# hellobertrand/zxc

Measured on NVIDIA H100. Metric: decompress GB/s (uncompressed), higher is better.
Workload: dtype u8

## Files before the change

profiles/occupancy_probe.py:

```python
import argparse
import ctypes as C
import os
import re
import shutil
import subprocess
import sys
import tempfile
import time

ROOT = os.path.dirname(os.path.dirname(os.path.abspath(__file__)))
sys.path.insert(0, os.path.join(ROOT, "tests"))
sys.path.insert(0, ROOT)

VARIANTS = [
    ("parent", "parent", "", {}, "shipped: lean at 8 CTAs, 64 registers without spills"),
    ("cta7", "cta7", "-DLEAN_CTAS_PER_SM=7u", {}, "the same source built for 7 CTAs (72 registers)"),
    ("grid7", "parent", "", {"ZXC_B200_DECODE_CTAS": "7"},
     "the shipped build with a 7-CTA grid: the eighth CTA alone, at the 164 KB carve-out"),
    ("pad7", "pad7", "-DLEAN_CTAS_PER_SM=7u -DLEAN_SMEM_PAD=2048u", {},
     "7 CTAs, 164 KB carve-out: the L1 shrink alone"),
    ("ring2k_7", "ring2k_7", "-DRING_BYTES=2048u -DLEAN_CTAS_PER_SM=7u", {}, "7 CTAs, 2 KiB rings"),
    ("ring2k_8", "ring2k_8", "-DRING_BYTES=2048u", {}, "8 CTAs, 2 KiB rings: more warps at a 100 KB carve-out"),
]
LEAN = "_Z17zxc_decode_kernelILb0ELb0ELb0ELb1EEv12DecodeParams"


def build(out_dir, nvextra):
    lib = os.path.join(out_dir, "libzxc.so.4")
    if not os.path.exists(lib):
        subprocess.run(["make", "-j", str(os.cpu_count() or 4), f"NVEXTRA={nvextra}", f"OUT={out_dir}"],
                       cwd=os.path.join(ROOT, "zxc_b200", "csrc"), check=True, stdout=subprocess.DEVNULL)
    return lib


def lean_resources(out_dir):
    log = open(os.path.join(out_dir, "obj", "ptxas.log")).read()
    blk = log.split(f"Compiling entry function '{LEAN}'")[1].split("Compiling entry function")[0]
    sp = re.search(r"(\d+) bytes spill stores, (\d+) bytes spill loads", blk)
    return int(re.search(r"Used (\d+) registers", blk).group(1)), int(sp.group(1)), int(sp.group(2))


def card():
    q = "name,power.limit,clocks.max.sm,clocks.sm"
    r = subprocess.run(["nvidia-smi", f"--query-gpu={q}", "--format=csv,noheader"], stdout=subprocess.PIPE, text=True)
    return r.stdout.strip().splitlines()[0] if r.returncode == 0 and r.stdout.strip() else "nvidia-smi unavailable"


class Runner:
    def __init__(self, path, dev, d_src, d_dst, d_jobs, d_status, nb):
        import bench
        import torch

        lib = C.CDLL(path)
        lib.zxc_b200_decode_scratch_size.restype = C.c_size_t
        lib.zxc_b200_decode_scratch_size.argtypes = [C.c_uint32]
        lib.zxc_b200_decode_blocks.restype = C.c_int
        lib.zxc_b200_decode_blocks.argtypes = [C.c_void_p, C.c_void_p, C.c_void_p, C.c_uint32, C.c_void_p,
                                               C.c_void_p, C.c_uint32, C.c_void_p, C.c_void_p, C.c_size_t,
                                               C.c_uint32, C.c_int, C.c_void_p]
        self.lib, self.nb, self.block = lib, nb, bench.BLOCK
        self.bufs = (d_src, d_dst, d_jobs, d_status)
        self.scratch_size = lib.zxc_b200_decode_scratch_size(bench.BLOCK)
        self.d_scratch = torch.empty(self.scratch_size, dtype=torch.uint8, device=dev)
        self.stream = torch.cuda.current_stream(dev)
        lean, general = C.c_int(0), C.c_int(0)
        assert lib.zxc_b200_decode_occupancy(C.byref(lean), C.byref(general)) == 0
        self.occupancy = (lean.value, general.value)

# ... 103 lines not shown
```

zxc_b200/csrc/zxc_decode.cuh:

```cuda
#pragma once
#include <cuda_runtime.h>
#include <stdint.h>

#include <type_traits>

#include "zxc_b200.h"
#include "zxc_error.h"

typedef uint8_t u8;
typedef uint32_t u32;
typedef uint64_t u64;
typedef int32_t i32;

#define FULL 0xFFFFFFFFu
#ifndef ZXC_FASTMOD
#define ZXC_FASTMOD 1
#endif
#ifndef ZXC_TAIL_SMEM
#define ZXC_TAIL_SMEM 1
#endif
#ifndef ZXC_ALIGNED_LD
#define ZXC_ALIGNED_LD 1
#endif
#ifndef ZXC_HINTS
// ... 96 lines not shown
__device__ __forceinline__ u8* ring_at(u32 a) { return reinterpret_cast<u8*>(__cvta_shared_to_generic((size_t)opaque(a))); }
__device__ __forceinline__ u32 grid_warp_now() {
    u32 t, c;
    asm volatile("mov.u32 %0, %%tid.x;" : "=r"(t));
    asm volatile("mov.u32 %0, %%ctaid.x;" : "=r"(c));
    return c * WARPS_PER_CTA + (t >> 5);
}
#else
extern u8 smem[];
static inline u32 smem_addr(const void* p) { return (u32)(reinterpret_cast<const u8*>(p) - smem); }
static inline u32 opaque(u32 v) { return v; }
static inline u8* ring_at(u32 a) { return smem + a; }
static inline u32 grid_warp_now() { return blockIdx.x * WARPS_PER_CTA + (threadIdx.x >> 5); }
template <int OFF> static inline void sts32(u32 a, u32 v) { memcpy(smem + a + OFF, &v, 4); }
template <int OFF> static inline void sts16(u32 a, u32 v) { const unsigned short h = (unsigned short)v; memcpy(smem + a + OFF, &h, 2); }
template <int OFF> static inline void sts8(u32 a, u32 v) { smem[a + OFF] = (u8)v; }
#endif

#ifdef __CUDACC__
__device__ __forceinline__ void prefetch_l1(const void* p) { asm volatile("prefetch.global.L1 [%0];" ::"l"(p)); }
#else
static inline void prefetch_l1(const void*) {}
#endif

#if ZXC_TRACE
#define TRACE_SLOTS 16
#define TRACE_ROWS 8192
enum {
    TR_UNPACK, TR_SCAN, TR_LIT, TR_MATCH, TR_TAIL, TR_FLUSH, TR_START, TR_END, TR_GIANT, TR_CLAIM,
    TR_BATCHES, TR_BLOCKS, TR_M_RING, TR_M_GLOBAL, TR_M_DICT, TR_M_SEQ
};
__device__ unsigned long long zxc_trace_acc[TRACE_ROWS * TRACE_SLOTS];
__device__ __forceinline__ void trace_add(u32 slot, unsigned long long v, u32 lane) {
    const u32 row = blockIdx.x * WARPS_PER_CTA + (threadIdx.x >> 5);
    if (lane == 0 && row < TRACE_ROWS) atomicAdd(&zxc_trace_acc[row * TRACE_SLOTS + slot], v);
}
#define ZXC_TRACE_DECL long long tr_t = clock64()
#define ZXC_TRACE_MARK(slot, lane)                               \
    do {                                                         \
        const long long tr_n = clock64();                        \
        trace_add(slot, (unsigned long long)(tr_n - tr_t), lane); \
        tr_t = tr_n;                                             \
    } while (0)
#define ZXC_TRACE_ADD(slot, v, lane) trace_add(slot, (unsigned long long)(v), lane)
#else
#define ZXC_TRACE_DECL
#define ZXC_TRACE_MARK(slot, lane)
#define ZXC_TRACE_ADD(slot, v, lane)
#endif

#include "zxc_decode_stage.cuh"
#define WARP_SMEM_BYTES (RING_BYTES + STAGE_BYTES)
#define DECODE_SMEM_BYTES (WARPS_PER_CTA * WARP_SMEM_BYTES)

#include "zxc_huffman.cuh"

__host__ __device__ __forceinline__ u32 scr_lit_cap(u32 bs) { return (bs + 255u) & ~255u; }
__host__ __device__ __forceinline__ u32 scr_tok_cap(u32 bs) { return (bs / 4u + 64u + 255u) & ~255u; }
__host__ __device__ __forceinline__ u32 scr_cum_cap(u32 bs) {
    return (11u * (scr_lit_cap(bs) / 8u) + 4u * 512u + 255u) & ~255u;
}
__host__ __device__ __forceinline__ u32 scr_stride(u32 bs) {
    return 256u + scr_lit_cap(bs) + scr_tok_cap(bs) + (u32)HUF_WORK_BYTES + scr_cum_cap(bs);
}

__device__ __forceinline__ void warp_copy(u8* d, const u8* s, u32 n, u32 lane) {
    u32 k = lane;
    for (; k + 96 < n; k += 128) {
        const u8 a = s[k], b = s[k + 32], c = s[k + 64], e = s[k + 96];
        d[k] = a;
        d[k + 32] = b;
        d[k + 64] = c;
        d[k + 96] = e;
    }
    for (; k < n; k += 32) d[k] = s[k];
}

__device__ __forceinline__ u32 read_varint(const u8* e, u32& pos, u32 end) {
    if (pos >= end) return 0;
    const u32 b0 = e[pos];
    if (b0 < 0x80) {
        pos += 1;
        return b0;
    }
    if (b0 < 0xC0) {
        if (pos + 1 >= end) {
            pos = end;
            return 0;
        }
        const u32 v = (b0 & 0x3F) | ((u32)e[pos + 1] << 6);
        pos += 2;
        return v;
    }
    if (b0 < 0xE0) {
        if (pos + 2 >= end) {
            pos = end;
            return 0;
        }
        const u32 v = (b0 & 0x1F) | ((u32)e[pos + 1] << 5) | ((u32)e[pos + 2] << 13);
        pos += 3;
        return v;
    }
    pos = end;
    return 0;
}

// ... 383 lines not shown
    const u32 total = __shfl_sync(FULL, incl, 31);
    const u32 excl = incl - c;
    const u32 pk = (my_d & (RING_BYTES - 1)) | (my_n << 16);
    const unsigned long long my_sp64 = reinterpret_cast<unsigned long long>(my_sp);
    for (u32 base = 0; base < total; base += 32) {
        ZXC_STAT(8, 1);
        const u32 q = base + lane;
        const bool act = q < total;
        u32 lo = 0, hi = 31;
#pragma unroll
        for (int it = 0; it < 5; it++) {
            const u32 mid = (lo + hi) >> 1;
            const u32 v = __shfl_sync(FULL, incl, mid);
            if (v > q) hi = mid;
            else lo = mid + 1;
        }
        const u32 j = lo & 31u;
        const u32 k = q - __shfl_sync(FULL, excl, j);
        const u32 pj = __shfl_sync(FULL, pk, j);
        const u8* sp = reinterpret_cast<const u8*>(__shfl_sync(FULL, my_sp64, j));
        if (act) {
            const u32 da = pj & 3u;
            const u32 n = pj >> 16;
            const u32 lfe = (da + n) >> 2;
            const u32 w0 = (da ? 1u : 0u) + 4u * k;
            const u8* bp = sp - da;
            const u32 m = (u32)(reinterpret_cast<uintptr_t>(bp)) & 3u;
            const u32* wp = reinterpret_cast<const u32*>(bp - m) + w0;
            const u32 dw = ring_s + (pj & 0xFFFFu) - da + 4u * w0;
            const u32 sh = m * 8u;
            const u32 left = lfe - w0;
            const u32 nsrc = left + (m ? 1u : 0u);
            u32 W[5];
#pragma unroll
            for (int i = 0; i < 5; i++) W[i] = (u32)i < nsrc ? wp[i] : 0u;
            sts32<0>(dw, __funnelshift_r(W[0], W[1], sh));
            if (1 < left) sts32<4>(dw, __funnelshift_r(W[1], W[2], sh));
            if (2 < left) sts32<8>(dw, __funnelshift_r(W[2], W[3], sh));
            if (3 < left) sts32<12>(dw, __funnelshift_r(W[3], W[4], sh));
        }
    }
}

#ifndef ZXC_NW
#define ZXC_NW 8
#endif
#define LIT_SHORT (4u * ZXC_NW - 4u)
#define MATCH_SHORT (4u * ZXC_NW - 4u)

__device__ __forceinline__ u32* esc_table(u8* scratch, u32 block_cap) {
    return reinterpret_cast<u32*>(scratch + scr_lit_cap(block_cap) + scr_tok_cap(block_cap) + (u32)HUF_WORK_BYTES);
}

template <bool UNITS, bool GHI, bool HAS_DICT, bool LEAN>
__device__ int decode_lz_block(const u8* pay, u32 comp, u8* out, u32 cap, const u8* dict_in,
                               u32 dict_size_in, const u8* dict_huf, u8* scratch, u32 scratch_cap, u8* ring,
                               u32 lane, const DecodeParams& P) {
    constexpr bool ghi = GHI;
    const u8* dict = HAS_DICT ? dict_in : (const u8*)0;
    const u32 dict_size = HAS_DICT ? dict_size_in : 0u;
    ZXC_TRACE_DECL;
    ZXC_TRACE_ADD(TR_BLOCKS, 1, lane);
    Sections S;
    const int prc = parse_sections<LEAN>(pay, comp, ghi, cap, dict_huf, scratch, scratch_cap, lane, S);
    if (prc != ZXC_OK) return prc;
    const u8* lit = S.lit;
    const u8* tok = S.tok;
    const u8* offs = S.offs;
    const u8* ext = S.ext;
    const u32 ext_end = S.ext_end, n_lit_avail = S.n_lit_avail, n_seq = S.n_seq, enc_off = S.enc_off;

    if (UNITS && cap <= 65536u) {
        u8* tok_buf = scratch + scr_lit_cap(scratch_cap);
        u8* hw_area = tok_buf + scr_tok_cap(scratch_cap);
        const bool scratch_busy = (lit == scratch) || (tok == tok_buf);
        u8* tab = scratch_busy ? hw_area : scratch;
        const u32 tab_bytes = scratch_busy ? (u32)HUF_WORK_BYTES + scr_cum_cap(scratch_cap)
                                           : scr_stride(scratch_cap) - 256u;
        const int r = decode_lz_units(lit, n_lit_avail, tok, offs, ext, ext_end, n_seq, enc_off, ghi, out, cap, dict,
                                      dict_size, tab, tab_bytes, lane);
        if (r != UW_NOT_TAKEN) return r;
    }

    const u32 mask = RING_BYTES - 1;
    const u32 esc = ghi ? 255u : 15u;
    const u32 lt_mask = (1u << lane) - 1u;
    const bool al16 = (reinterpret_cast<uintptr_t>(out) & 15u) == 0;
    Window w;
    w.ring = ring;
    w.out = out;
    w.dict = dict;
    w.dict_size = dict_size;
    w.near_lo = 0;
    const u32 ring_s = smem_addr(ring);
    (void)ring_s;
#define W_RING()                                     \
    do {                                             \
        if constexpr (LEAN) w.ring = ring_at(ring_s); \
    } while (0)
    u32 O = 0, L = 0, F = 0, epos = 0, ring_lo = 0;

    u32* vals = esc_table(scratch, scratch_cap);
    if constexpr (LEAN) {
        if (4ull * ext_end > scr_cum_cap(scratch_cap)) return D2_DEFER_STATUS;
    }
    const bool use_vals = LEAN || (ext_end != 0u && 4ull * ext_end <= scr_cum_cap(scratch_cap));
    u32 n_val = 0, ord_base = 0;
    if (use_vals && (!LEAN || ext_end != 0u)) {
        const u32 seg = max(4u, (ext_end + 31u) / 32u);
        const u32 nseg = (ext_end + seg - 1u) / seg;
        const u32 lo = lane * seg, hi = min(ext_end, lo + seg);
        u64 inc = lane < nseg ? z2_seg_map(ext, lo, hi, ext_end) : Z2_MAP_ID;
#pragma unroll
        for (int dd = 1; dd < 32; dd <<= 1) {
            const u64 o = __shfl_up_sync(FULL, inc, dd);
            if (lane >= (u32)dd) inc = z2_map_compose(o, inc);
        }
        u64 excl = __shfl_up_sync(FULL, inc, 1);
        if (lane == 0) excl = Z2_MAP_ID;
        n_val = z2_map_cnt(__shfl_sync(FULL, inc, 31), 0);
        if (lane < nseg) {
            const u32 ent = z2_map_exit(excl, 0);
            if (ent != 3u) z2_seg_values(ext, lo, hi, ext_end, ent, z2_map_cnt(excl, 0), vals);
        }
        __syncwarp();
    }

#if ZXC_STAGE
    const u32 stage_s = smem_addr(ring) + RING_BYTES;
    TokStream::open(stage_s, tok, (ghi ? 4u : 1u) * n_seq, pay + comp, tok >= pay && tok < pay + comp);
    OffStream::open(stage_s, ghi ? tok : offs, ghi ? 0u : (enc_off ? 1u : 2u) * n_seq, pay + comp, !ghi);
#if ZXC_STAGE_LIT
    LitStream::open(stage_s, lit, n_lit_avail, pay + comp, lit >= pay && lit < pay + comp);
#define ST_LIT_CLOSE() LitStream::close(stage_s)
#else
#define ST_LIT_CLOSE() do { } while (0)
#endif
#define ST_CLOSE()                   \
    do {                             \
        TokStream::close(stage_s);   \
        OffStream::close(stage_s);   \
        ST_LIT_CLOSE();              \
    } while (0)
#else
#define ST_CLOSE() do { } while (0)
#define ST_LIT_CLOSE() do { } while (0)
#endif

    ZXC_TRACE_MARK(TR_START, lane);

    u32 base = 0;
    while (base < n_seq) {
        const u32 i = base + lane;
        const bool valid = i < n_seq;
        u32 ll = 0, ml = 0, off = 1;
        if (LEAN && !HAS_DICT && lane < 4u && L + 128u * lane < n_lit_avail) prefetch_l1(lit + L + 128u * lane);
#if ZXC_STAGE
        const u32 tok_w = ghi ? 4u : 1u, off_w = enc_off ? 1u : 2u;
        const u32 tx0 = (u32)(reinterpret_cast<uintptr_t>(tok) & 15u), ox0 = (u32)(reinterpret_cast<uintptr_t>(offs) & 15u);
        const u32 i_end = min(base + 32u, n_seq);
        const StWindow st_t = TokStream::need(stage_s, tok, tx0 + tok_w * base, tx0 + tok_w * i_end, 0u, lane);
        const StWindow st_o = OffStream::need(stage_s, offs, ox0 + off_w * base, ox0 + off_w * i_end, 0u, lane);
        const bool t_st = tx0 + tok_w * i_end <= st_t.hi, o_st = !ghi && ox0 + off_w * i_end <= st_o.hi;
#endif
        if (valid) {
            u32 a, b = 0;
#if ZXC_STAGE
            if (!ghi) {
                a = t_st ? lds8(st_t.ring_s + ((tx0 + i) & (ST_RING - 1u))) : (u32)tok[i];
                if (!o_st) {
                    b = enc_off ? (u32)offs[i] : ld16(offs + 2 * (size_t)i);
                } else if (enc_off) {
                    b = lds8(st_o.ring_s + ((ox0 + i) & (ST_RING - 1u)));
                } else {
                    const u32 x = ox0 + 2u * i;
                    b = (ox0 & 1u) ? (lds8(st_o.ring_s + (x & (ST_RING - 1u))) |
                                      (lds8(st_o.ring_s + ((x + 1u) & (ST_RING - 1u))) << 8))
                                   : lds16(st_o.ring_s + (x & (ST_RING - 1u)));
                }
            } else if (t_st) {
                const u32 x = tx0 + 4u * i;
                if (tx0 & 3u) {
                    a = lds8(st_t.ring_s + (x & (ST_RING - 1u))) | (lds8(st_t.ring_s + ((x + 1u) & (ST_RING - 1u))) << 8) |
                        (lds8(st_t.ring_s + ((x + 2u) & (ST_RING - 1u))) << 16) |
                        (lds8(st_t.ring_s + ((x + 3u) & (ST_RING - 1u))) << 24);
                } else {
                    a = lds32(st_t.ring_s + (x & (ST_RING - 1u)));
                }
            } else {
                a = ld32(tok + 4 * (size_t)i);
            }
#else
            if (!ghi) {
                const u8* tk = tok;
                if constexpr (LEAN) tk = lit + opaque(n_lit_avail);
                a = tk[i];
#if ZXC_ALIGNED_LD
                if (LEAN) {
                    const u32 oi = n_seq + (enc_off ? i : 2u * i);
                    if (enc_off) b = (u32)tk[oi];
                    else if ((reinterpret_cast<uintptr_t>(tk) + n_seq) & 1u) b = ld16(tk + oi);
                    else b = (u32)*reinterpret_cast<const unsigned short*>(tk + oi);
                } else if (enc_off) b = (u32)offs[i];
                else if (reinterpret_cast<uintptr_t>(offs) & 1u) b = ld16(offs + 2 * (size_t)i);
                else b = (u32)reinterpret_cast<const unsigned short*>(offs)[i];
#else
                b = enc_off ? (u32)offs[i] : ld16(offs + 2 * (size_t)i);
#endif
            } else {
#if ZXC_ALIGNED_LD
                a = (reinterpret_cast<uintptr_t>(tok) & 3u) ? ld32(tok + 4 * (size_t)i) : reinterpret_cast<const u32*>(tok)[i];
#else
                a = ld32(tok + 4 * (size_t)i);
#endif
            }
#endif
            if (!ghi) {
                ll = a >> 4;
                ml = a & 15;
                off = b + 1;
            } else {
                ll = a >> 24;
                ml = (a >> 16) & 0xFF;
                off = (a & 0xFFFF) + 1;
            }
        }
        const bool e_ll = valid && ll == esc, e_ml = valid && ml == esc;
        const u32 m_ll = __ballot_sync(FULL, e_ll), m_ml = __ballot_sync(FULL, e_ml);
        ZXC_TRACE_MARK(TR_UNPACK, lane);
        u32 k_esc = 0, epos_end = epos;
        if ((m_ll | m_ml) && use_vals) {
            const u32* vt = vals;
            if constexpr (LEAN) vt = esc_table(warp_scratch(P, grid_warp_now()), P.block_cap);
            u32 k = ord_base + __popc(m_ll & lt_mask) + __popc(m_ml & lt_mask);
            if (e_ll) {
                ll += k < n_val ? vt[k] : 0u;
                k++;
            }
            if (e_ml) ml += k < n_val ? vt[k] : 0u;
        } else if (ZXC_RARE((m_ll | m_ml) != 0)) {
            const u32 ord_ll = __popc(m_ll & lt_mask) + __popc(m_ml & lt_mask);
            k_esc = __popc(m_ll) + __popc(m_ml);
            u32 my_pos = ext_end;
            for (u32 s = 0; s < k_esc; s++) {
                if (s == ord_ll) my_pos = epos_end;
                epos_end = varint_advance(ext, epos_end, ext_end);
            }
            if (e_ll) ll += read_varint(ext, my_pos, ext_end);
            if (e_ml) ml += read_varint(ext, my_pos, ext_end);
        }
        if (valid) ml += 5;
        const u32 tot = ll + ml;
        const u32 s_ll = warp_incl_scan(ll, lane);
        const u32 s_tot = warp_incl_scan(tot, lane);

        const u32 nvalid = min(32u, n_seq - base);
        const u32 m = __popc(__ballot_sync(FULL, valid && s_tot <= RING_LIMIT));
        const u32 lit_start = L + s_ll - ll;
        const u32 out_start = O + s_tot - tot;
        const u32 mdst = out_start + ll;

        if (ZXC_RARE(m == 0)) {
            const u32 g_ll = __shfl_sync(FULL, ll, 0), g_ml = __shfl_sync(FULL, ml, 0),
                      g_off = __shfl_sync(FULL, off, 0);
            ZXC_STAT(9, 1);
            if (L + g_ll > n_lit_avail || (u64)O + g_ll + g_ml > cap) {
                ST_CLOSE();
                return ZXC_ERROR_OVERFLOW;
            }
            if (O + g_ll + dict_size < g_off) {
                ST_CLOSE();
                return ZXC_ERROR_BAD_OFFSET;
            }
            __syncwarp();
            W_RING();
            ring_flush(w, F, O, lane, al16);
            __syncwarp();
            flush_wait(lane);
            warp_copy(out + O, lit + L, g_ll, lane);
            __syncwarp();
            warp_match_global(w, O + g_ll, g_off, g_ml, lane);
            __syncwarp();
            O += g_ll + g_ml;
            L += g_ll;
            F = O;
            ring_lo = O >= 64 ? O - 64 : 0;
            for (u32 p = ring_lo + lane; p < O; p += 32) w.ring[p & mask] = out[p];
            __syncwarp();
            const u32 q = ((m_ll & 1u) ? 1u : 0u) + ((m_ml & 1u) ? 1u : 0u);
            ord_base += q;
            if (!use_vals)
                for (u32 s = 0; s < q; s++) epos = varint_advance(ext, epos, ext_end);
            base += 1;
            ZXC_TRACE_MARK(TR_GIANT, lane);
            continue;
        }

        ZXC_STAT(10, m < nvalid);
        ZXC_STAT(11, m < nvalid && !use_vals);
        const bool act = lane < m;
        const bool ovf = act && (lit_start + ll > n_lit_avail || out_start + tot > cap);
        const bool bad = act && (mdst + dict_size < off);
        const u32 m_err = __ballot_sync(FULL, ovf || bad);
        if (ZXC_RARE(m_err != 0)) {
            ZXC_STAT(19, 1);
            const int code = ovf ? ZXC_ERROR_OVERFLOW : ZXC_ERROR_BAD_OFFSET;
            ST_CLOSE();
            return __shfl_sync(FULL, code, __ffs(m_err) - 1);
        }
        const u32 T = __shfl_sync(FULL, s_tot, m - 1), TL = __shfl_sync(FULL, s_ll, m - 1);
#if ZXC_STAGE && ZXC_STAGE_LIT
        const u32 lx0 = (u32)(reinterpret_cast<uintptr_t>(lit) & 15u);
        const StWindow lw = LitStream::need(stage_s, lit, lx0 + L, lx0 + L + TL, 8u, lane);
#endif
        {
            const i32 a = (i32)(O + T) - (i32)RING_BYTES + 32;
            w.near_lo = a > (i32)ring_lo ? a : (i32)ring_lo;
        }

        flush_wait(lane);
        const i32 src_lo = (i32)mdst - (i32)off;
        const i32 src_end = min((i32)mdst, src_lo + (i32)ml);
        const bool near = src_lo >= w.near_lo;
        const u32 si = (u32)src_lo & mask;
        const bool in_dict = src_lo + (i32)ml + 8 <= 0 && (i32)dict_size + src_lo >= 8;
        const bool m_word_ok = ((mdst & mask) + ml + 4 <= RING_BYTES) &&
                               (near ? (si >= 8 && si + ml + 8 <= RING_BYTES)
                                     : (in_dict || (src_lo >= 8 && src_lo + (i32)ml + 4 <= w.near_lo)));
        const bool m_lane_ok = m_word_ok && ml <= MATCH_SHORT && off >= ml;
        const bool m_grp_ok = m_word_ok && !m_lane_ok && off >= ml;
        auto match_src = [&]() -> const u8* {
            return near ? (LEAN ? ring_at(ring_s + si) : ring + si)
                        : (src_lo < 0 ? dict + ((i32)dict_size + src_lo) : out + src_lo);
        };
        const u8* m_sp = LEAN ? nullptr : match_src();
        const bool l_word_ok = (out_start & mask) + ll + 4 <= RING_BYTES;

        const bool m_free = src_end <= (i32)O;
        if (LEAN && !HAS_DICT && act && m_free && !near && src_lo >= 0) {
            const u8* ps = out + src_lo;
            const u8* pe = ps + ml - 1u;
            prefetch_l1(ps);
            if ((reinterpret_cast<uintptr_t>(ps) ^ reinterpret_cast<uintptr_t>(pe)) >> 7) prefetch_l1(pe);
        }
        ZXC_TRACE_ADD(TR_M_RING, __popc(__ballot_sync(FULL, act && near)), lane);
        ZXC_TRACE_ADD(TR_M_GLOBAL, __popc(__ballot_sync(FULL, act && !near && src_lo >= 0)), lane);
        ZXC_TRACE_ADD(TR_M_DICT, __popc(__ballot_sync(FULL, act && !near && src_lo < 0)), lane);
        ZXC_TRACE_ADD(TR_M_SEQ, __popc(__ballot_sync(FULL, act && !m_free)), lane);
        ZXC_TRACE_ADD(TR_BATCHES, 1, lane);
        ZXC_TRACE_MARK(TR_SCAN, lane);
        ZXC_STAT(0, 1);
        ZXC_STAT(1, m);
        bool lit_pass = true;
#pragma unroll 1
        for (;;) {
            bool ready, lok, gok;
            u32 it_d, it_n;
            const u8* it_sp;
            if (lit_pass) {
                ready = act && ll > 0;
                it_d = out_start;
                it_n = ll;
                it_sp = lit + lit_start;
// ... 28 lines not shown
            ZXC_STAT(20, __popc(__ballot_sync(FULL, !lit_pass && ready && (lok || gok) && near)));
            ZXC_STAT(21, __popc(__ballot_sync(FULL, !lit_pass && ready && (lok || gok) && !near && src_lo >= 0)));
            if (m_grp) balanced_copy_words(ring_s, m_grp, it_d, it_sp, it_n, lane);
            u32 m_slow = __ballot_sync(FULL, ready && !lok && !gok);
            while (ZXC_RARE(m_slow != 0)) {
                const int j = __ffs(m_slow) - 1;
                m_slow &= m_slow - 1;
                const u32 d = __shfl_sync(FULL, it_d, j), n = __shfl_sync(FULL, it_n, j);
                const u32 aux = __shfl_sync(FULL, lit_pass ? lit_start : off, j);
                W_RING();
                if (lit_pass) {
                    for (u32 k = lane; k < n; k += 32) w.ring[(d + k) & mask] = lit[aux + k];
                } else {
                    warp_match_to_ring(w, d, aux, n, lane);
                }
            }
            __syncwarp();
            ZXC_TRACE_MARK(lit_pass ? TR_LIT : TR_MATCH, lane);
            if (!lit_pass) break;
            lit_pass = false;
        }
        {
            u32 rest = __ballot_sync(FULL, act && !m_free);
            const u32 my_pk = ml | ((near && off >= ml) ? 0x80000000u : 0u);
            ZXC_STAT(12, __popc(rest));
            while (rest) {
                const int j = __ffs(rest) - 1;
                rest &= rest - 1;
                const u32 d = __shfl_sync(FULL, mdst, j), pk = __shfl_sync(FULL, my_pk, j);
                const u32 n = pk & 0x7FFFFFFFu;
                if (pk >> 31) {
                    const u32 sl = __shfl_sync(FULL, (u32)src_lo, j);
#if ZXC_TAIL_SMEM
                    for (u32 k = lane; k < n; k += 32) sts8<0>(ring_s + ((d + k) & mask), lds8(ring_s + ((sl + k) & mask)));
#else
                    for (u32 k = lane; k < n; k += 32) ring[(d + k) & mask] = ring[(sl + k) & mask];
#endif
                } else {
                    W_RING();
                    warp_match_to_ring(w, d, __shfl_sync(FULL, off, j), n, lane);
                }
                __syncwarp();
            }
        }
        ZXC_TRACE_MARK(TR_TAIL, lane);

        O += T;
        L += TL;
        W_RING();
        ring_flush(w, F, O & ~511u, lane, al16);
        __syncwarp();
        ZXC_TRACE_MARK(TR_FLUSH, lane);

        if (m < nvalid) {
            const u32 below = (1u << m) - 1u;
            const u32 q = __popc(m_ll & below) + __popc(m_ml & below);
            ord_base += q;
            if (!use_vals)
                for (u32 s = 0; s < q; s++) epos = varint_advance(ext, epos, ext_end);
            base += m;
        } else {
            ord_base += __popc(m_ll) + __popc(m_ml);
            epos = epos_end;
            base += 32;
        }
    }

    ST_LIT_CLOSE();
    const u32 rem = n_lit_avail - L;
    if (rem > cap - O) return ZXC_ERROR_OVERFLOW;
    W_RING();
#undef W_RING
    ring_flush(w, F, O, lane, al16);
    __syncwarp();
    flush_wait(lane);
    warp_copy(out + O, lit + L, rem, lane);
    ZXC_TRACE_MARK(TR_END, lane);
    return (int)(O + rem);
}

template <bool UNITS, bool HAS_DICT, bool LEAN = false>
__device__ int decode_job(const DecodeParams& P, const zxc_b200_job_t& job, u8* scratch, u8* ring, u32 lane) {
    const u8* blk = P.src + job.src_off;
    u8* out = P.dst + job.dst_off;
    if (job.src_len < 8) return LEAN ? D2_DEFER_STATUS : ZXC_ERROR_SRC_TOO_SMALL;
    const u32 type = blk[0];
    const u32 comp = ld32(blk + 3);
    const bool verify = (P.flags & FLAG_VERIFY) != 0;
    if (LEAN) {
        const bool whole = !verify && (u64)job.src_len >= 8ull + comp;
        const bool take = whole && (type == BT_RAW || (type == BT_GLO && comp >= 12u && blk[8 + 9] == 0 && blk[8 + 8] <= 1));
        if (!take) return D2_DEFER_STATUS;
    }
    if ((u64)job.src_len < 8ull + comp + (verify ? 4u : 0u)) return ZXC_ERROR_SRC_TOO_SMALL;
    const u8* data = blk + 8;
    if constexpr (!LEAN) {
        if (verify && ld32(data + comp) != warp_checksum(data, comp, lane)) return ZXC_ERROR_BAD_CHECKSUM;
    }
    switch (type) {
        case BT_GLO:
            return decode_lz_block<UNITS, false, HAS_DICT, LEAN>(data, comp, out, job.dst_cap, P.dict, P.dict_size,
                                                                 P.dict_huf, scratch, P.block_cap, ring, lane, P);
        case BT_GHI:
            if constexpr (LEAN) return D2_DEFER_STATUS;
            else return decode_lz_block<UNITS, true, HAS_DICT, false>(data, comp, out, job.dst_cap, P.dict, P.dict_size,
                                                                      P.dict_huf, scratch, P.block_cap, ring, lane, P);
        case BT_RAW:
            if (comp > job.dst_cap) return ZXC_ERROR_DST_TOO_SMALL;
            warp_copy(out, data, comp, lane);
            return (int)comp;
        case BT_EOF:
            return ZXC_ERROR_CORRUPT_DATA;
        default:
            return ZXC_ERROR_BAD_BLOCK_TYPE;
    }
}

template <bool UNITS, bool DEFERRED, bool HAS_DICT, bool LEAN>
__global__ void __launch_bounds__(CTA_THREADS, LEAN ? LEAN_CTAS_PER_SM : CTAS_PER_SM) zxc_decode_kernel(const DecodeParams P) {
    extern __shared__ __align__(16) u8 smem[];
    const u32 lane = threadIdx.x & 31;
    const u32 wic = threadIdx.x >> 5;
    const u32 gwarp = blockIdx.x * WARPS_PER_CTA + wic;
    u8* scratch = warp_scratch(P, gwarp);
    u8* ring = smem + (size_t)wic * WARP_SMEM_BYTES;
#if ZXC_STAGE
    st_init(smem_addr(ring) + RING_BYTES, lane);
#endif
    if (DEFERRED) {
        const u32 n_def = *P.defer_count;
        if (n_def == 0) return;
        if (n_def <= P.defer_cap) {
            for (;;) {
                unsigned long long k = 0;
                if (lane == 0) k = atomicAdd(P.counter, 1ull);
                k = __shfl_sync(FULL, k, 0);
                if (k >= n_def) break;
                const u32 j = P.defer_list[k];
                const zxc_b200_job_t job = P.jobs[j];
                const int r = decode_job<UNITS, HAS_DICT, false>(P, job, scratch, ring, lane);
                flush_wait(lane);
                __syncwarp();
                if (lane == 0) P.status[j] = r;
            }
            return;
        }
        for (;;) {
            unsigned long long b = 0;
            if (lane == 0) b = atomicAdd(P.counter, 32ull);
            b = __shfl_sync(FULL, b, 0);
            if (b >= P.n_jobs) break;
            const unsigned long long jj = b + lane;
            u32 m = __ballot_sync(FULL, jj < P.n_jobs && P.status[jj] == D2_DEFER_STATUS);
            while (m) {
                const unsigned long long j = b + (u32)(__ffs(m) - 1);
                m &= m - 1;
                const zxc_b200_job_t job = P.jobs[j];
                const int r = decode_job<UNITS, HAS_DICT, false>(P, job, scratch, ring, lane);
                flush_wait(lane);
                __syncwarp();
                if (lane == 0) P.status[j] = r;
            }
        }
        return;
    }
    using JobIx = typename std::conditional<LEAN, u32, unsigned long long>::type;
    u32 ring_s = 0;
    if constexpr (LEAN) ring_s = smem_addr(ring);
    for (;;) {
        ZXC_TRACE_DECL;
        unsigned long long c = 0;
        if (lane == 0) c = atomicAdd(P.counter, 1ull);
        const JobIx j = __shfl_sync(FULL, (JobIx)c, 0);
        ZXC_TRACE_MARK(TR_CLAIM, lane);
        if (j >= P.n_jobs) break;
        const zxc_b200_job_t job = P.jobs[j];
        const int r = LEAN ? decode_job<UNITS, HAS_DICT, LEAN>(P, job, warp_scratch(P, grid_warp_now()), ring_at(ring_s), lane)
                           : decode_job<UNITS, HAS_DICT, LEAN>(P, job, scratch, ring, lane);
// ... 32 lines not shown
```

zxc_b200/csrc/zxc_gpu.cu:

```cuda
#include <cuda_runtime.h>
#include <stdint.h>
#include <stdio.h>
#include <stdlib.h>
#include <string.h>
#include <pthread.h>

#include "zxc_error.h"
#include "zxc_gpu.h"

#include "zxc_decode.cuh"
#include "zxc_decode2.cuh"
#include "zxc_encode.cuh"
#include "zxc_assemble.cuh"
#include "zxc_dplan.cuh"
#include "zxc_train.cuh"

static pthread_once_t g_once = PTHREAD_ONCE_INIT;
static int g_init_rc = ZXC_B200_ERROR_NO_DEVICE;
static int g_sm_count = 0;
static unsigned long long g_launches = 0;
static pthread_mutex_t g_pool_mu = PTHREAD_MUTEX_INITIALIZER;

#define PIN_CHUNK ((size_t)32 << 20)

// ... 230 lines not shown
    unsigned long long* reduce_out;
    cudaStream_t s_h2d, s_d2h;
    cudaStream_t s_dec[STAGE_SLOTS];
    cudaEvent_t ev_ring[EV_RING];
    pinned_buf st_in[STAGE_SLOTS], st_out[STAGE_SLOTS];
    cudaEvent_t st_ev_in[STAGE_SLOTS], st_ev_dec[STAGE_SLOTS], st_ev_out[STAGE_SLOTS];
    int st_ready;
    struct zxg_ctx* next;
    int device;
    int numa_node;
    int sm_count;
    int trimmed;
};
static zxg_ctx* g_free_list = NULL;

static void init_once(void) {
    int n = 0;
    const cudaError_t e = cudaGetDeviceCount(&n);
    if (e != cudaSuccess || n <= 0) {
        fprintf(stderr,
                "libzxc (CUDA build): no usable CUDA device (%s); this library has no CPU codec, "
                "codec entry points return ZXC_B200_ERROR_NO_DEVICE\n",
                e != cudaSuccess ? cudaGetErrorString(e) : "device count 0");
        g_init_rc = ZXC_B200_ERROR_NO_DEVICE;
        return;
    }
    int dev = 0;
    cudaGetDevice(&dev);
    cudaDeviceProp prop;
    if (cudaGetDeviceProperties(&prop, dev) != cudaSuccess) {
        g_init_rc = ZXC_B200_ERROR_CUDA;
        return;
    }
    g_sm_count = prop.multiProcessorCount;
    g_init_rc = ZXC_OK;
}

extern "C" int zxg_init(void) {
    pthread_once(&g_once, init_once);
    return g_init_rc;
}

extern "C" int zxc_b200_device_count(void) {
    int n = 0;
    if (cudaGetDeviceCount(&n) != cudaSuccess) return 0;
    return n;
}

extern "C" uint64_t zxc_b200_launch_count(void) { return g_launches; }

extern "C" int zxc_b200_decode_occupancy(int* lean, int* general) {
    if (zxg_init() != ZXC_OK) return ZXC_B200_ERROR_CUDA;
    if (cudaOccupancyMaxActiveBlocksPerMultiprocessor(lean, zxc_decode_kernel<false, false, false, true>, CTA_THREADS,
                                                      DECODE_SMEM_BYTES + LEAN_SMEM_PAD) != cudaSuccess ||
        cudaOccupancyMaxActiveBlocksPerMultiprocessor(general, zxc_decode_kernel<false, true, false, false>, CTA_THREADS,
                                                      DECODE_SMEM_BYTES) != cudaSuccess)
        return ZXC_B200_ERROR_CUDA;
    return ZXC_OK;
}

#if ZXC_TRACE
extern "C" ZXC_EXPORT int zxc_b200_trace_read(unsigned long long* host) {
    const size_t bytes = sizeof(unsigned long long) * TRACE_ROWS * TRACE_SLOTS;
    if (cudaDeviceSynchronize() != cudaSuccess) return -1;
    if (cudaMemcpyFromSymbol(host, zxc_trace_acc, bytes) != cudaSuccess) return -1;
    void* d = 0;
    if (cudaGetSymbolAddress(&d, zxc_trace_acc) != cudaSuccess || cudaMemset(d, 0, bytes) != cudaSuccess) return -1;
    if (cudaDeviceSynchronize() != cudaSuccess) return -1;
    return TRACE_ROWS * TRACE_SLOTS;
}
#endif

extern "C" int zxg_current_device(void) {
    int dev = 0;
    if (cudaGetDevice(&dev) != cudaSuccess) {
        cudaGetLastError();
        return 0;
    }
    return dev;
}
extern "C" int zxg_device_count(void) { return zxc_b200_device_count(); }
extern "C" int zxg_set_device(int dev) {
    if (cudaSetDevice(dev) != cudaSuccess) {
        cudaGetLastError();
        return ZXC_B200_ERROR_CUDA;
    }
    return ZXC_OK;
}

extern "C" zxg_ctx* zxg_create(void) {
    if (zxg_init() != ZXC_OK) return NULL;
    zxg_ctx* c = (zxg_ctx*)calloc(1, sizeof(zxg_ctx));
    if (!c) return NULL;
    cudaGetDevice(&c->device);
    if (cudaStreamCreateWithFlags(&c->stream, cudaStreamNonBlocking) != cudaSuccess ||
        cudaMalloc((void**)&c->counter, 32 * sizeof(unsigned long long)) != cudaSuccess) {
        free(c);
        return NULL;
    }
    c->reduce_out = c->counter + 28;
    c->numa_node = device_numa_node(c->device);
    int smc = 0;
    if (cudaDeviceGetAttribute(&smc, cudaDevAttrMultiProcessorCount, c->device) != cudaSuccess || smc <= 0) smc = g_sm_count;
    c->sm_count = smc;
    return c;
}

// ... 319 lines not shown
        Q.defer_cap = P.defer_cap;
        Q.defer_list = P.defer_list;
        Q.trace = NULL;
        const int want_trace = getenv("ZXC_B200_D2_TRACE") != NULL;
        if (want_trace && cudaMalloc((void**)&Q.trace, (size_t)n_jobs * 128) == cudaSuccess)
            cudaMemsetAsync(Q.trace, 0, (size_t)n_jobs * 128, st);
        zxc_decode2_kernel<<<grid2, c.threads, c.smem, st>>>(Q);
        __atomic_add_fetch(&g_launches, 1, __ATOMIC_RELAXED);
        if (cudaGetLastError() != cudaSuccess) return ZXC_B200_ERROR_CUDA;
        if (Q.trace) {
            unsigned long long* h = (unsigned long long*)malloc((size_t)n_jobs * 128);
            cudaStreamSynchronize(st);
            cudaMemcpy(h, Q.trace, (size_t)n_jobs * 128, cudaMemcpyDeviceToHost);
            double acc[6] = {0, 0, 0, 0, 0, 0};
            u32 cnt = 0;
            for (u32 i = 0; i < n_jobs; i++) {
                const unsigned long long* t = h + (size_t)i * 8;
                if (!t[6] || !t[5]) continue;
                for (int q = 0; q < 6; q++) acc[q] += (double)(t[q + 1] - t[q]);
                cnt++;
            }
            if (cnt)
                fprintf(stderr, "d2 trace (%u blocks, mean cycles): header+issue %.0f | load wait %.0f | extras %.0f | records %.0f | "
                                "words %.0f | drain %.0f\n", cnt, acc[0] / cnt, acc[1] / cnt, acc[2] / cnt, acc[3] / cnt,
                        acc[4] / cnt, acc[5] / cnt);
            double w[8] = {0, 0, 0, 0, 0, 0, 0, 0};
            for (u32 i = 0; i < n_jobs; i++) {
                const unsigned long long* t = h + (size_t)i * 8;
                if (!t[6] || !t[5]) continue;
                for (int q = 0; q < 8; q++) w[q] += (double)h[(size_t)n_jobs * 8 + (size_t)i * 8 + q];
            }
            if (cnt)
                fprintf(stderr, "d2 trace warp 0 per block: steps %.1f rounds %.1f sleeps %.1f | cycles: guard %.0f plan %.0f rounds %.0f "
                                "sleep %.0f finish %.0f\n", w[7] / cnt, w[5] / cnt, w[6] / cnt, w[0] / cnt, w[1] / cnt, w[2] / cnt,
                        w[3] / cnt, w[4] / cnt);
            free(h);
            cudaFree(Q.trace);
        }
        P.flags |= FLAG_DEFERRED;
        P.counter = d_counter + 1;
    }
    const bool has_dict = P.dict != NULL && P.dict_size != 0;
    if (!verify && !units && !(P.flags & FLAG_DEFERRED)) {
#ifdef LEAN_CARVEOUT
        static int carveout_done = 0;
        if (!carveout_done) {
            cudaFuncSetAttribute(zxc_decode_kernel<false, false, true, true>,
                                 cudaFuncAttributePreferredSharedMemoryCarveout, LEAN_CARVEOUT);
            cudaFuncSetAttribute(zxc_decode_kernel<false, false, false, true>,
                                 cudaFuncAttributePreferredSharedMemoryCarveout, LEAN_CARVEOUT);
            carveout_done = 1;
        }
#endif
        const u32 lean_smem = DECODE_SMEM_BYTES + LEAN_SMEM_PAD;
        if (has_dict) zxc_decode_kernel<false, false, true, true><<<grid, CTA_THREADS, lean_smem, st>>>(P);
        else zxc_decode_kernel<false, false, false, true><<<grid, CTA_THREADS, lean_smem, st>>>(P);
        __atomic_add_fetch(&g_launches, 1, __ATOMIC_RELAXED);
        if (cudaGetLastError() != cudaSuccess) return ZXC_B200_ERROR_CUDA;
        P.flags |= FLAG_DEFERRED;
        P.counter = d_counter + 1;
    }
    {
        const int resident = (g_sm_count > 0 ? g_sm_count : 132) * (int)CTAS_PER_SM;
        if (grid > resident) grid = resident;
    }
    if (P.flags & FLAG_DEFERRED) {
        if (has_dict) zxc_decode_kernel<false, true, true, false><<<grid, CTA_THREADS, DECODE_SMEM_BYTES, st>>>(P);
        else zxc_decode_kernel<false, true, false, false><<<grid, CTA_THREADS, DECODE_SMEM_BYTES, st>>>(P);
    } else if (units) {
        if (has_dict) zxc_decode_kernel<true, false, true, false><<<grid, CTA_THREADS, DECODE_SMEM_BYTES, st>>>(P);
        else zxc_decode_kernel<true, false, false, false><<<grid, CTA_THREADS, DECODE_SMEM_BYTES, st>>>(P);
    } else {
        if (has_dict) zxc_decode_kernel<false, false, true, false><<<grid, CTA_THREADS, DECODE_SMEM_BYTES, st>>>(P);
        else zxc_decode_kernel<false, false, false, false><<<grid, CTA_THREADS, DECODE_SMEM_BYTES, st>>>(P);
    }
    __atomic_add_fetch(&g_launches, 1, __ATOMIC_RELAXED);
    return cudaGetLastError() == cudaSuccess ? ZXC_OK : ZXC_B200_ERROR_CUDA;
}

static int launch_decode(const void* d_src, void* d_dst, const zxc_b200_job_t* d_jobs, u32 n_jobs,
                         i32* d_status, const void* d_dict, u32 dict_size, const void* d_dict_huf,
                         void* d_scratch, size_t scratch_size, u32 block_size, int verify,
                         unsigned long long* d_counter, cudaStream_t st) {
    return launch_decode_ex(d_src, d_dst, d_jobs, n_jobs, d_status, d_dict, dict_size, d_dict_huf, d_scratch,
                            scratch_size, block_size, verify, d_counter, st, 0);
}

static size_t launch_scratch_bytes(u32 n_jobs, u32 block_size) {
    size_t n = (size_t)grid_for(n_jobs) * WARPS_PER_CTA * scratch_stride_for(block_size);
    n = (n + 255) & ~(size_t)255;
    D2Config c;
    if (d2_config(block_size, &c) && c.spill_stride) n = (n + d2_spill_bytes(&c) + 255) & ~(size_t)255;
    return n + (size_t)DEFER_CAP * 4 + 256;
}

extern "C" int zxc_b200_decode_blocks(const void* d_src, void* d_dst, const zxc_b200_job_t* d_jobs,
                                      uint32_t n_jobs, int32_t* d_status, const void* d_dict,
                                      uint32_t dict_size, const void* d_dict_huf, void* d_scratch,
                                      size_t scratch_size, uint32_t block_size, int verify_checksums,
                                      void* stream) {
    const int rc = zxg_init();
    if (rc != ZXC_OK) return rc;
    if (!d_src || !d_dst || !d_jobs || !d_status || !d_scratch) return ZXC_ERROR_NULL_INPUT;
    if (scratch_size < SCRATCH_TAIL) return ZXC_ERROR_MEMORY;
    const size_t usable = (scratch_size - SCRATCH_TAIL) & ~(size_t)7;
    unsigned long long* counter = (unsigned long long*)((u8*)d_scratch + usable);
    return launch_decode(d_src, d_dst, d_jobs, n_jobs, d_status, d_dict, dict_size, d_dict_huf,
// ... 1026 lines not shown
```

Measured before the change: 431.4.

## Prefetch next batch's tokens, offsets and escapes into a per-warp cp.async slot

Adds a per-warp 256-byte shared-memory look-ahead slot in the lean no-dictionary decode path. While the current batch of sequences is processed, cp.async copies the next batch's token bytes, offset words and escape values into that slot. The next iteration then reads them from shared memory instead of issuing dependent global loads at the top of the batch. This is meant to hide global load latency, at the cost of extra shared memory per warp (which may affect CTAs per SM), more registers, and a wait_all per batch.

```diff
diff --git a/profiles/occupancy_probe.py b/profiles/occupancy_probe.py
--- a/profiles/occupancy_probe.py
+++ b/profiles/occupancy_probe.py
@@ -13,7 +13,9 @@
 sys.path.insert(0, ROOT)
 
 VARIANTS = [
-    ("parent", "parent", "", {}, "shipped: lean at 8 CTAs, 64 registers without spills"),
+    ("parent", "parent", "", {}, "shipped: lean at 8 CTAs, 64 registers without spills, look-ahead slot"),
+    ("lookahead0", "lookahead0", "-DZXC_LOOKAHEAD=0", {},
+     "the lean instances without the look-ahead slot (tokens, offsets, escapes loaded at the batch top)"),
     ("cta7", "cta7", "-DLEAN_CTAS_PER_SM=7u", {}, "the same source built for 7 CTAs (72 registers)"),
     ("grid7", "parent", "", {"ZXC_B200_DECODE_CTAS": "7"},
      "the shipped build with a 7-CTA grid: the eighth CTA alone, at the 164 KB carve-out"),
diff --git a/zxc_b200/csrc/zxc_decode.cuh b/zxc_b200/csrc/zxc_decode.cuh
--- a/zxc_b200/csrc/zxc_decode.cuh
+++ b/zxc_b200/csrc/zxc_decode.cuh
@@ -172,6 +172,55 @@
 #include "zxc_decode_stage.cuh"
 #define WARP_SMEM_BYTES (RING_BYTES + STAGE_BYTES)
 #define DECODE_SMEM_BYTES (WARPS_PER_CTA * WARP_SMEM_BYTES)
+
+#ifndef ZXC_LOOKAHEAD
+#define ZXC_LOOKAHEAD (!ZXC_STAGE)
+#endif
+#if ZXC_LOOKAHEAD && ZXC_STAGE
+#error "ZXC_LOOKAHEAD and ZXC_STAGE both stage the token and offset sections: build with one of them"
+#endif
+#define LA_SLOT_BYTES (ZXC_LOOKAHEAD ? 256u : 0u)
+#define LA_OFF 48u
+#define LA_ESC 128u
+#define LEAN_WARP_SMEM_BYTES (WARP_SMEM_BYTES + LA_SLOT_BYTES)
+#define LEAN_SMEM_BYTES (WARPS_PER_CTA * LEAN_WARP_SMEM_BYTES + LEAN_SMEM_PAD)
+template <bool HAS_DICT, bool LEAN> __host__ __device__ constexpr bool la_on() {
+    return LEAN && !HAS_DICT && ZXC_LOOKAHEAD != 0;
+}
+
+#ifdef __CUDACC__
+__device__ __forceinline__ void cp_async4(u32 sdst, const void* gsrc) {
+    asm volatile("cp.async.ca.shared.global [%0], [%1], 4;" ::"r"(sdst), "l"(gsrc) : "memory");
+}
+__device__ __forceinline__ void cp_async_wait_all() { asm volatile("cp.async.wait_all;" ::: "memory"); }
+__device__ __forceinline__ void cp_async_check_idle() {}
+#else
+struct SimtCpAsync {
+    u32 s;
+    const u8* g;
+};
+inline SimtCpAsync simt_cp_pending[32][8];
+inline u32 simt_cp_n[32];
+static inline void simt_cp_fail(const char* what) {
+    fprintf(stderr, "simt cp.async check failed: %s\n", what);
+    abort();
+}
+static inline void cp_async4(u32 sdst, const void* gsrc) {
+    const int l = simt::g_warp->current;
+    if ((sdst & 3u) || (reinterpret_cast<uintptr_t>(gsrc) & 3u)) simt_cp_fail("4-byte copy not 4-byte aligned");
+    if (simt_cp_n[l] >= 8) simt_cp_fail("more copies in flight than a lane issues per batch");
+    memset(smem + sdst, 0xE7, 4);
+    simt_cp_pending[l][simt_cp_n[l]++] = SimtCpAsync{sdst, static_cast<const u8*>(gsrc)};
+}
+static inline void cp_async_wait_all() {
+    const int l = simt::g_warp->current;
+    for (u32 k = 0; k < simt_cp_n[l]; k++) memcpy(smem + simt_cp_pending[l][k].s, simt_cp_pending[l][k].g, 4);
+    simt_cp_n[l] = 0;
+}
+static inline void cp_async_check_idle() {
+    if (simt_cp_n[simt::g_warp->current]) simt_cp_fail("a copy was still in flight when the previous block ended");
+}
+#endif
 
 #include "zxc_huffman.cuh"
 
@@ -661,6 +710,27 @@
     return reinterpret_cast<u32*>(scratch + scr_lit_cap(block_cap) + scr_tok_cap(block_cap) + (u32)HUF_WORK_BYTES);
 }
 
+__device__ __forceinline__ void la_issue_words(u32 slot_s, const u8* tk, u32 n_seq, u32 enc_off, u32 nb, u32 lane) {
+    if (nb < n_seq) {
+        const u32 nt = min(32u, n_seq - nb), ow = enc_off ? 1u : 2u;
+        const bool t = lane < LA_OFF / 4u;
+        const u8* s = t ? tk + nb : tk + n_seq + ow * nb;
+        const u32 n = t ? nt : ow * nt;
+        const u32 x = (u32)reinterpret_cast<uintptr_t>(s) & 3u;
+        const u32 k = t ? lane : lane - LA_OFF / 4u;
+        if (4u * k < x + n) cp_async4(slot_s + 4u * lane, s - x + 4u * k);
+    }
+}
+__device__ __forceinline__ void la_issue_esc(u32 slot_s, u32 n_val, u32 ob, u32 lane, const DecodeParams& P) {
+    if (ob + lane < n_val)
+        cp_async4(slot_s + LA_ESC + 4u * lane, esc_table(warp_scratch(P, grid_warp_now()), P.block_cap) + ob + lane);
+}
+__device__ __forceinline__ u32 la_esc(u32 slot_s, u32 k, u32 ob, u32 n_val, const DecodeParams& P) {
+    if (k >= n_val) return 0u;
+    if (k - ob < 32u) return lds32(slot_s + LA_ESC + 4u * (k - ob));
+    return esc_table(warp_scratch(P, grid_warp_now()), P.block_cap)[k];
+}
+
 template <bool UNITS, bool GHI, bool HAS_DICT, bool LEAN>
 __device__ int decode_lz_block(const u8* pay, u32 comp, u8* out, u32 cap, const u8* dict_in,
                                u32 dict_size_in, const u8* dict_huf, u8* scratch, u32 scratch_cap, u8* ring,
@@ -703,6 +773,9 @@
     w.near_lo = 0;
     const u32 ring_s = smem_addr(ring);
     (void)ring_s;
+    constexpr bool LA = la_on<HAS_DICT, LEAN>();
+    const u32 slot_s = ring_s + WARP_SMEM_BYTES;
+    (void)slot_s;
 #define W_RING()                                     \
     do {                                             \
         if constexpr (LEAN) w.ring = ring_at(ring_s); \
@@ -712,6 +785,10 @@
     u32* vals = esc_table(scratch, scratch_cap);
     if constexpr (LEAN) {
         if (4ull * ext_end > scr_cum_cap(scratch_cap)) return D2_DEFER_STATUS;
+    }
+    if constexpr (LA) {
+        cp_async_check_idle();
+        la_issue_words(slot_s, tok, n_seq, enc_off, 0u, lane);
     }
     const bool use_vals = LEAN || (ext_end != 0u && 4ull * ext_end <= scr_cum_cap(scratch_cap));
     u32 n_val = 0, ord_base = 0;
@@ -734,6 +811,7 @@
         }
         __syncwarp();
     }
+    if constexpr (LA) la_issue_esc(slot_s, n_val, 0u, lane, P);
 
 #if ZXC_STAGE
     const u32 stage_s = smem_addr(ring) + RING_BYTES;
@@ -764,6 +842,10 @@
         const bool valid = i < n_seq;
         u32 ll = 0, ml = 0, off = 1;
         if (LEAN && !HAS_DICT && lane < 4u && L + 128u * lane < n_lit_avail) prefetch_l1(lit + L + 128u * lane);
+        if constexpr (LA) {
+            cp_async_wait_all();
+            __syncwarp();
+        }
 #if ZXC_STAGE
         const u32 tok_w = ghi ? 4u : 1u, off_w = enc_off ? 1u : 2u;
         const u32 tx0 = (u32)(reinterpret_cast<uintptr_t>(tok) & 15u), ox0 = (u32)(reinterpret_cast<uintptr_t>(offs) & 15u);
@@ -803,19 +885,28 @@
             if (!ghi) {
                 const u8* tk = tok;
                 if constexpr (LEAN) tk = lit + opaque(n_lit_avail);
-                a = tk[i];
+                if constexpr (LA) {
+                    a = lds8(slot_s + ((u32)reinterpret_cast<uintptr_t>(tk + base) & 3u) + lane);
+                    const u32 ox = (u32)reinterpret_cast<uintptr_t>(tk + n_seq + (enc_off ? base : 2u * base)) & 3u;
+                    const u32 oa = slot_s + LA_OFF + ox + (enc_off ? lane : 2u * lane);
+                    if (enc_off) b = lds8(oa);
+                    else if (ox & 1u) b = lds8(oa) | (lds8(oa + 1u) << 8);
+                    else b = lds16(oa);
+                } else {
+                    a = tk[i];
 #if ZXC_ALIGNED_LD
-                if (LEAN) {
-                    const u32 oi = n_seq + (enc_off ? i : 2u * i);
-                    if (enc_off) b = (u32)tk[oi];
-                    else if ((reinterpret_cast<uintptr_t>(tk) + n_seq) & 1u) b = ld16(tk + oi);
-                    else b = (u32)*reinterpret_cast<const unsigned short*>(tk + oi);
-                } else if (enc_off) b = (u32)offs[i];
-                else if (reinterpret_cast<uintptr_t>(offs) & 1u) b = ld16(offs + 2 * (size_t)i);
-                else b = (u32)reinterpret_cast<const unsigned short*>(offs)[i];
+                    if (LEAN) {
+                        const u32 oi = n_seq + (enc_off ? i : 2u * i);
+                        if (enc_off) b = (u32)tk[oi];
+                        else if ((reinterpret_cast<uintptr_t>(tk) + n_seq) & 1u) b = ld16(tk + oi);
+                        else b = (u32)*reinterpret_cast<const unsigned short*>(tk + oi);
+                    } else if (enc_off) b = (u32)offs[i];
+                    else if (reinterpret_cast<uintptr_t>(offs) & 1u) b = ld16(offs + 2 * (size_t)i);
+                    else b = (u32)reinterpret_cast<const unsigned short*>(offs)[i];
 #else
-                b = enc_off ? (u32)offs[i] : ld16(offs + 2 * (size_t)i);
-#endif
+                    b = enc_off ? (u32)offs[i] : ld16(offs + 2 * (size_t)i);
+#endif
+                }
             } else {
 #if ZXC_ALIGNED_LD
                 a = (reinterpret_cast<uintptr_t>(tok) & 3u) ? ld32(tok + 4 * (size_t)i) : reinterpret_cast<const u32*>(tok)[i];
@@ -842,11 +933,19 @@
             const u32* vt = vals;
             if constexpr (LEAN) vt = esc_table(warp_scratch(P, grid_warp_now()), P.block_cap);
             u32 k = ord_base + __popc(m_ll & lt_mask) + __popc(m_ml & lt_mask);
-            if (e_ll) {
-                ll += k < n_val ? vt[k] : 0u;
-                k++;
-            }
-            if (e_ml) ml += k < n_val ? vt[k] : 0u;
+            if constexpr (LA) {
+                if (e_ll) {
+                    ll += la_esc(slot_s, k, ord_base, n_val, P);
+                    k++;
+                }
+                if (e_ml) ml += la_esc(slot_s, k, ord_base, n_val, P);
+            } else {
+                if (e_ll) {
+                    ll += k < n_val ? vt[k] : 0u;
+                    k++;
+                }
+                if (e_ml) ml += k < n_val ? vt[k] : 0u;
+            }
         } else if (ZXC_RARE((m_ll | m_ml) != 0)) {
             const u32 ord_ll = __popc(m_ll & lt_mask) + __popc(m_ml & lt_mask);
             k_esc = __popc(m_ll) + __popc(m_ml);
@@ -901,6 +1000,10 @@
             if (!use_vals)
                 for (u32 s = 0; s < q; s++) epos = varint_advance(ext, epos, ext_end);
             base += 1;
+            if constexpr (LA) {
+                la_issue_words(slot_s, lit + opaque(n_lit_avail), n_seq, enc_off, base, lane);
+                la_issue_esc(slot_s, n_val, ord_base, lane, P);
+            }
             ZXC_TRACE_MARK(TR_GIANT, lane);
             continue;
         }
@@ -918,6 +1021,13 @@
             return __shfl_sync(FULL, code, __ffs(m_err) - 1);
         }
         const u32 T = __shfl_sync(FULL, s_tot, m - 1), TL = __shfl_sync(FULL, s_ll, m - 1);
+        if constexpr (LA) {
+            const u32 below = m < 32u ? (1u << m) - 1u : FULL;
+            ord_base += __popc(m_ll & below) + __popc(m_ml & below);
+            base += m;
+            la_issue_words(slot_s, lit + opaque(n_lit_avail), n_seq, enc_off, base, lane);
+            la_issue_esc(slot_s, n_val, ord_base, lane, P);
+        }
 #if ZXC_STAGE && ZXC_STAGE_LIT
         const u32 lx0 = (u32)(reinterpret_cast<uintptr_t>(lit) & 15u);
         const StWindow lw = LitStream::need(stage_s, lit, lx0 + L, lx0 + L + TL, 8u, lane);
@@ -1052,7 +1162,8 @@
         __syncwarp();
         ZXC_TRACE_MARK(TR_FLUSH, lane);
 
-        if (m < nvalid) {
+        if constexpr (LA) {
+        } else if (m < nvalid) {
             const u32 below = (1u << m) - 1u;
             const u32 q = __popc(m_ll & below) + __popc(m_ml & below);
             ord_base += q;
@@ -1065,6 +1176,7 @@
             base += 32;
         }
     }
+    if constexpr (LA) cp_async_wait_all();
 
     ST_LIT_CLOSE();
     const u32 rem = n_lit_avail - L;
@@ -1123,7 +1235,7 @@
     const u32 wic = threadIdx.x >> 5;
     const u32 gwarp = blockIdx.x * WARPS_PER_CTA + wic;
     u8* scratch = warp_scratch(P, gwarp);
-    u8* ring = smem + (size_t)wic * WARP_SMEM_BYTES;
+    u8* ring = smem + (size_t)wic * (la_on<HAS_DICT, LEAN>() ? LEAN_WARP_SMEM_BYTES : WARP_SMEM_BYTES);
 #if ZXC_STAGE
     st_init(smem_addr(ring) + RING_BYTES, lane);
 #endif
diff --git a/zxc_b200/csrc/zxc_gpu.cu b/zxc_b200/csrc/zxc_gpu.cu
--- a/zxc_b200/csrc/zxc_gpu.cu
+++ b/zxc_b200/csrc/zxc_gpu.cu
@@ -306,7 +306,7 @@
 extern "C" int zxc_b200_decode_occupancy(int* lean, int* general) {
     if (zxg_init() != ZXC_OK) return ZXC_B200_ERROR_CUDA;
     if (cudaOccupancyMaxActiveBlocksPerMultiprocessor(lean, zxc_decode_kernel<false, false, false, true>, CTA_THREADS,
-                                                      DECODE_SMEM_BYTES + LEAN_SMEM_PAD) != cudaSuccess ||
+                                                      LEAN_SMEM_BYTES) != cudaSuccess ||
         cudaOccupancyMaxActiveBlocksPerMultiprocessor(general, zxc_decode_kernel<false, true, false, false>, CTA_THREADS,
                                                       DECODE_SMEM_BYTES) != cudaSuccess)
         return ZXC_B200_ERROR_CUDA;
@@ -732,7 +732,7 @@
             carveout_done = 1;
         }
 #endif
-        const u32 lean_smem = DECODE_SMEM_BYTES + LEAN_SMEM_PAD;
+        const u32 lean_smem = has_dict ? DECODE_SMEM_BYTES + LEAN_SMEM_PAD : LEAN_SMEM_BYTES;
         if (has_dict) zxc_decode_kernel<false, false, true, true><<<grid, CTA_THREADS, lean_smem, st>>>(P);
         else zxc_decode_kernel<false, false, false, true><<<grid, CTA_THREADS, lean_smem, st>>>(P);
         __atomic_add_fetch(&g_launches, 1, __ATOMIC_RELAXED);
```

New measurement: 458.2, median of 6. 1.06x the previous value.
